# yangdongchao/Text-to-sound-Synthesis

Hardware: NVIDIA H100
Metric: clips/sec (10s audio, 100 diffusion steps) (higher is better)
Workload: dtype f16x3

## Files before the change

text-to-sound-synthesis_b200/csrc/attention_tc_split.cu:

```cuda
#include "common.cuh"
#include "diffsound_b200.h"
#include <cuda_fp16.h>

namespace dsb {
namespace {
constexpr int SP_HD = 64;
constexpr int SP_KMAX = 288;
constexpr int SP_MAX_WARPS = 12;

struct SpParams {
  int B, H, Lq, Lk, kpad, box_rows, n_box;
  int slabs, slabs_per_cta;
  const __half* q;
  long long ldq;
  int q_lo_col, k_lo_col, v_lo_col;
  long long ldo, o_lo_off;
  __half* o;
  float scale_log2e;
};

__device__ __forceinline__ float sp_ex2(float x) {
  float y;
  asm("ex2.approx.ftz.f32 %0, %1;" : "=f"(y) : "f"(x));
  return y;
}

__device__ __forceinline__ uint32_t sp_sw128(int r, int chunk) { return r * 128 + ((chunk ^ (r & 7)) << 4); }
__device__ __forceinline__ void sp_ldsm_x4(uint32_t (&r)[4], const uint8_t* p) {
  asm volatile("ldmatrix.sync.aligned.m8n8.x4.shared.b16 {%0,%1,%2,%3}, [%4];" : "=r"(r[0]), "=r"(r[1]), "=r"(r[2]), "=r"(r[3]) : "r"(smem_u32(p)));
}
__device__ __forceinline__ void sp_ldsm_x4_t(uint32_t (&r)[4], const uint8_t* p) {
  asm volatile("ldmatrix.sync.aligned.m8n8.x4.trans.shared.b16 {%0,%1,%2,%3}, [%4];" : "=r"(r[0]), "=r"(r[1]), "=r"(r[2]), "=r"(r[3]) : "r"(smem_u32(p)));
}
__device__ __forceinline__ void sp_mma(float (&d)[4], const uint32_t (&a)[4], uint32_t b0, uint32_t b1) {
  asm volatile("mma.sync.aligned.m16n8k16.row.col.f32.f16.f16.f32 {%0,%1,%2,%3}, {%4,%5,%6,%7}, {%8,%9}, {%0,%1,%2,%3};"
               : "+f"(d[0]), "+f"(d[1]), "+f"(d[2]), "+f"(d[3])
               : "r"(a[0]), "r"(a[1]), "r"(a[2]), "r"(a[3]), "r"(b0), "r"(b1));
}
__device__ __forceinline__ void sp_pack_pair(float a, float b, uint32_t& hi, uint32_t& lo) {
  const __half2 h = __floats2half2_rn(a, b);
  const __half2 l = __floats2half2_rn(a - __low2float(h), b - __high2float(h));
  hi = *reinterpret_cast<const uint32_t*>(&h);
  lo = *reinterpret_cast<const uint32_t*>(&l);
}
__device__ __forceinline__ void sp_remainder_rows(const SpParams& p, const uint8_t* sKh, const uint8_t* sKl, const uint8_t* sVh, const uint8_t* sVl, int b, int h,
                                                  int row0, int lane) {
  const int g = lane >> 2, t = lane & 3;
  const __half* qb = p.q + (long long)b * p.Lq * p.ldq + h * SP_HD;
  uint32_t ah[4][4], al[4][4];
#pragma unroll
  for (int ks = 0; ks < 4; ++ks) {
    const int ra = row0 + g, rb = row0 + g + 8, c = ks * 16 + 2 * t;
    const __half* pa = qb + (long long)ra * p.ldq + c;
    const __half* pb = qb + (long long)rb * p.ldq + c;
    ah[ks][0] = ra < p.Lq ? *reinterpret_cast<const uint32_t*>(pa) : 0u;
    ah[ks][1] = rb < p.Lq ? *reinterpret_cast<const uint32_t*>(pb) : 0u;
    ah[ks][2] = ra < p.Lq ? *reinterpret_cast<const uint32_t*>(pa + 8) : 0u;
    ah[ks][3] = rb < p.Lq ? *reinterpret_cast<const uint32_t*>(pb + 8) : 0u;
    al[ks][0] = ra < p.Lq ? *reinterpret_cast<const uint32_t*>(pa + p.q_lo_col) : 0u;
    al[ks][1] = rb < p.Lq ? *reinterpret_cast<const uint32_t*>(pb + p.q_lo_col) : 0u;
    al[ks][2] = ra < p.Lq ? *reinterpret_cast<const uint32_t*>(pa + p.q_lo_col + 8) : 0u;
    al[ks][3] = rb < p.Lq ? *reinterpret_cast<const uint32_t*>(pb + p.q_lo_col + 8) : 0u;
  }
  float m0 = -INFINITY, m1 = -INFINITY, l0 = 0.f, l1 = 0.f;
  float oacc[8][4];
#pragma unroll
  for (int i = 0; i < 8; ++i) oacc[i][0] = oacc[i][1] = oacc[i][2] = oacc[i][3] = 0.f;
  for (int kc = 0; kc * 64 < p.kpad; ++kc) {
    const int keys_left = p.Lk - kc * 64;
    if (keys_left <= 0) break;
    const int n_live = keys_left >= 64 ? 8 : (keys_left + 7) >> 3;
    float s[8][4];
#pragma unroll
    for (int nt = 0; nt < 8; ++nt) {
      s[nt][0] = s[nt][1] = s[nt][2] = s[nt][3] = 0.f;
      if (nt >= n_live) continue;
      const int row = kc * 64 + nt * 8 + (lane & 7);
      uint32_t kh[4], kl[4];
#pragma unroll
      for (int half = 0; half < 2; ++half) {
        sp_ldsm_x4(kh, sKh + sp_sw128(row, 4 * half + (lane >> 3)));
        sp_ldsm_x4(kl, sKl + sp_sw128(row, 4 * half + (lane >> 3)));
        sp_mma(s[nt], al[2 * half], kh[0], kh[1]);
        sp_mma(s[nt], al[2 * half + 1], kh[2], kh[3]);
        sp_mma(s[nt], ah[2 * half], kl[0], kl[1]);
        sp_mma(s[nt], ah[2 * half + 1], kl[2], kl[3]);
        sp_mma(s[nt], ah[2 * half], kh[0], kh[1]);
        sp_mma(s[nt], ah[2 * half + 1], kh[2], kh[3]);
      }
    }
    float mx0 = -INFINITY, mx1 = -INFINITY;
#pragma unroll
    for (int nt = 0; nt < 8; ++nt) {
      const int key = kc * 64 + nt * 8 + 2 * t;
      if (key >= p.Lk) { s[nt][0] = -INFINITY; s[nt][2] = -INFINITY; }
      if (key + 1 >= p.Lk) { s[nt][1] = -INFINITY; s[nt][3] = -INFINITY; }
      mx0 = fmaxf(mx0, fmaxf(s[nt][0], s[nt][1]));
      mx1 = fmaxf(mx1, fmaxf(s[nt][2], s[nt][3]));
    }
    mx0 = fmaxf(mx0, __shfl_xor_sync(0xffffffffu, mx0, 1)); mx0 = fmaxf(mx0, __shfl_xor_sync(0xffffffffu, mx0, 2));
    mx1 = fmaxf(mx1, __shfl_xor_sync(0xffffffffu, mx1, 1)); mx1 = fmaxf(mx1, __shfl_xor_sync(0xffffffffu, mx1, 2));
    const float mn0 = fmaxf(m0, mx0), mn1 = fmaxf(m1, mx1);
    const float c0 = sp_ex2((m0 - mn0) * p.scale_log2e), c1 = sp_ex2((m1 - mn1) * p.scale_log2e);
    const float ms0 = mn0 * p.scale_log2e, ms1 = mn1 * p.scale_log2e;
    m0 = mn0; m1 = mn1;
    l0 *= c0; l1 *= c1;
#pragma unroll
    for (int nd = 0; nd < 8; ++nd) { oacc[nd][0] *= c0; oacc[nd][1] *= c0; oacc[nd][2] *= c1; oacc[nd][3] *= c1; }
#pragma unroll
    for (int nt = 0; nt < 8; ++nt) {
      s[nt][0] = sp_ex2(fmaf(s[nt][0], p.scale_log2e, -ms0)); s[nt][1] = sp_ex2(fmaf(s[nt][1], p.scale_log2e, -ms0));
      s[nt][2] = sp_ex2(fmaf(s[nt][2], p.scale_log2e, -ms1)); s[nt][3] = sp_ex2(fmaf(s[nt][3], p.scale_log2e, -ms1));
      l0 += s[nt][0] + s[nt][1];
      l1 += s[nt][2] + s[nt][3];
    }
#pragma unroll
    for (int kk = 0; kk < 4; ++kk) {
      if (kk * 2 >= n_live) continue;
      uint32_t ph[4], pl[4];
      sp_pack_pair(s[2 * kk][0], s[2 * kk][1], ph[0], pl[0]);
      sp_pack_pair(s[2 * kk][2], s[2 * kk][3], ph[1], pl[1]);
      sp_pack_pair(s[2 * kk + 1][0], s[2 * kk + 1][1], ph[2], pl[2]);
      sp_pack_pair(s[2 * kk + 1][2], s[2 * kk + 1][3], ph[3], pl[3]);
      const int row = kc * 64 + kk * 16 + (lane & 7) + 8 * ((lane >> 3) & 1);
#pragma unroll
      for (int np = 0; np < 4; ++np) {
        uint32_t vh[4], vl[4];
        sp_ldsm_x4_t(vh, sVh + sp_sw128(row, 2 * np + (lane >> 4)));
        sp_ldsm_x4_t(vl, sVl + sp_sw128(row, 2 * np + (lane >> 4)));
        sp_mma(oacc[2 * np], pl, vh[0], vh[1]);
        sp_mma(oacc[2 * np + 1], pl, vh[2], vh[3]);
        sp_mma(oacc[2 * np], ph, vl[0], vl[1]);
        sp_mma(oacc[2 * np + 1], ph, vl[2], vl[3]);
        sp_mma(oacc[2 * np], ph, vh[0], vh[1]);
        sp_mma(oacc[2 * np + 1], ph, vh[2], vh[3]);
      }
    }
  }
  l0 += __shfl_xor_sync(0xffffffffu, l0, 1); l0 += __shfl_xor_sync(0xffffffffu, l0, 2);
  l1 += __shfl_xor_sync(0xffffffffu, l1, 1); l1 += __shfl_xor_sync(0xffffffffu, l1, 2);
  const float i0 = 1.0f / l0, i1 = 1.0f / l1;
  const int ra = row0 + g, rb = row0 + g + 8;
  __half* ob = p.o + (long long)b * p.Lq * p.ldo + h * SP_HD;
#pragma unroll
  for (int nd = 0; nd < 8; ++nd) {
    uint32_t hi, lo;
    if (ra < p.Lq) {
      sp_pack_pair(oacc[nd][0] * i0, oacc[nd][1] * i0, hi, lo);
      *reinterpret_cast<uint32_t*>(ob + (long long)ra * p.ldo + nd * 8 + 2 * t) = hi;
      *reinterpret_cast<uint32_t*>(ob + (long long)ra * p.ldo + p.o_lo_off + nd * 8 + 2 * t) = lo;
    }
    if (rb < p.Lq) {
      sp_pack_pair(oacc[nd][2] * i1, oacc[nd][3] * i1, hi, lo);
      *reinterpret_cast<uint32_t*>(ob + (long long)rb * p.ldo + nd * 8 + 2 * t) = hi;
      *reinterpret_cast<uint32_t*>(ob + (long long)rb * p.ldo + p.o_lo_off + nd * 8 + 2 * t) = lo;
    }
  }
}

__global__ void __launch_bounds__(SP_MAX_WARPS * 32, 1)
attention_tc_split_kernel(const __grid_constant__ CUtensorMap map_k, const __grid_constant__ CUtensorMap map_v, const __grid_constant__ SpParams p) {
  extern __shared__ uint8_t smem_raw[];
  uint8_t* smem = reinterpret_cast<uint8_t*>((reinterpret_cast<uintptr_t>(smem_raw) + 1023) & ~uintptr_t(1023));
  const int kv_bytes = p.kpad * 128;
  uint8_t* sKh = smem;
  uint8_t* sKl = sKh + kv_bytes;
  uint8_t* sVh = sKl + kv_bytes;
  uint8_t* sVl = sVh + kv_bytes;
  uint64_t* kv_full = reinterpret_cast<uint64_t*>(sVl + kv_bytes);
  const int u = blockIdx.x, b = u / p.H, h = u - b * p.H;
  const int warp = threadIdx.x >> 5, lane = threadIdx.x & 31;

  if (threadIdx.x == 0) {
    mbar_init(kv_full, 1);
    fence_barrier_init();
    prefetch_tmap(&map_k); prefetch_tmap(&map_v);
  }
  __syncthreads();
  pdl_wait();
  pdl_trigger();
  if (threadIdx.x == 0) {
    mbar_arrive_expect_tx(kv_full, 4 * kv_bytes);
    for (int bx = 0; bx < p.n_box; ++bx) {
      const int r = b * p.Lk + bx * p.box_rows, off = bx * p.box_rows * 128;
      tma_load_3d(&map_k, kv_full, sKh + off, h * SP_HD, r, 0);
      tma_load_3d(&map_k, kv_full, sKl + off, p.k_lo_col + h * SP_HD, r, 0);
      tma_load_3d(&map_v, kv_full, sVh + off, h * SP_HD, r, 0);
      tma_load_3d(&map_v, kv_full, sVl + off, p.v_lo_col + h * SP_HD, r, 0);
    }
  }
  mbar_wait(kv_full, 0);
  const int s0 = blockIdx.y * p.slabs_per_cta, s1 = min(p.slabs, s0 + p.slabs_per_cta);
  for (int sl = s0 + warp; sl < s1; sl += blockDim.x >> 5) sp_remainder_rows(p, sKh, sKl, sVh, sVl, b, h, sl * 16, lane);
}
}
}

extern "C" int dsb_attention_tc_split(const void* q, long long ldq, long long q_lo_off, const void* k, long long ldk, long long k_lo_off, const void* v,
                                      long long ldv, long long v_lo_off, void* o, long long ldo, long long o_lo_off, int B, int H, int Lq, int Lk,
                                      float scale, void* stream) {
  using namespace dsb;
  DSB_REQUIRE(B > 0 && H > 0 && Lq > 0 && Lk > 0 && Lk <= SP_KMAX, "dsb_attention_tc_split: need 0 < Lk <= %d", SP_KMAX);
  DSB_REQUIRE(ldo % 8 == 0 && o_lo_off % 8 == 0 && (reinterpret_cast<uintptr_t>(o) & 15) == 0, "dsb_attention_tc_split: o must be 16-byte aligned, ldo / o_lo_off %% 8 == 0");
  DSB_REQUIRE(q_lo_off >= (long long)H * SP_HD && k_lo_off >= (long long)H * SP_HD && v_lo_off >= (long long)H * SP_HD && o_lo_off >= (long long)H * SP_HD,
              "dsb_attention_tc_split: the lo halves must not overlap the hi halves");
  DSB_REQUIRE(q_lo_off + (long long)H * SP_HD <= ldq && k_lo_off + (long long)H * SP_HD <= ldk && v_lo_off + (long long)H * SP_HD <= ldv,
              "dsb_attention_tc_split: lo halves must lie inside a row (lo_off + H*64 <= ld)");
  DSB_REQUIRE(ldq % 2 == 0 && q_lo_off % 2 == 0 && (reinterpret_cast<uintptr_t>(q) & 3) == 0, "dsb_attention_tc_split: q must be 4-byte aligned");
  SpParams p{};
  p.B = B; p.H = H; p.Lq = Lq; p.Lk = Lk;
  p.kpad = (Lk + 31) & ~31;
  p.q = (const __half*)q; p.ldq = ldq;
  p.n_box = p.kpad > 256 ? 2 : 1;
  p.box_rows = p.kpad / p.n_box;
  DSB_REQUIRE(p.box_rows % 8 == 0, "dsb_attention_tc_split: internal box size");
  p.q_lo_col = (int)q_lo_off; p.k_lo_col = (int)k_lo_off; p.v_lo_col = (int)v_lo_off;
  p.ldo = ldo; p.o_lo_off = o_lo_off; p.o = (__half*)o;
  p.scale_log2e = scale * 1.4426950408889634f;
  p.slabs = (Lq + 15) / 16;
  const int ny = (p.slabs + SP_MAX_WARPS - 1) / SP_MAX_WARPS;
  p.slabs_per_cta = (p.slabs + ny - 1) / ny;
  CUtensorMap mk, mv;
  if (make_operand_map(&mk, k, DSB_DTYPE_F16, k_lo_off + (long long)H * SP_HD, (long long)B * Lk, 1, ldk, 0, p.box_rows)) return 3;
  if (make_operand_map(&mv, v, DSB_DTYPE_F16, v_lo_off + (long long)H * SP_HD, (long long)B * Lk, 1, ldv, 0, p.box_rows)) return 3;
  const int smem = 4 * p.kpad * 128 + 8 + 1024;
  static int attr_smem = 0;
  if (smem > attr_smem) {
    DSB_CHECK_CUDA(cudaFuncSetAttribute(attention_tc_split_kernel, cudaFuncAttributeMaxDynamicSharedMemorySize, smem));
    attr_smem = smem;
  }
  DSB_CHECK_CUDA(launch_pdl(attention_tc_split_kernel, dim3(B * H, ny), dim3(p.slabs_per_cta * 32), smem, (cudaStream_t)stream, mk, mv, p));
  return 0;
}
```

text-to-sound-synthesis_b200/csrc/wgmma.cuh:

```cuda
#pragma once
#include "common.cuh"
#include "diffsound_b200.h"

namespace dsb {

template <int KIND, int TA, int TB>
__device__ __forceinline__ void wgmma_m64n128(float (&d)[64], uint64_t da, uint64_t db, uint32_t scale_d) {
  static_assert(KIND != DSB_DTYPE_TF32 || (TA == 0 && TB == 0), "tf32 wgmma takes K-major operands only");
  if constexpr (KIND == DSB_DTYPE_TF32) {
    asm volatile(
        "{\n\t.reg .pred p;\n\tsetp.ne.b32 p, %66, 0;\n\t"
        "wgmma.mma_async.sync.aligned.m64n128k8.f32.tf32.tf32 "
        "{%0, %1, %2, %3, %4, %5, %6, %7, %8, %9, %10, %11, %12, %13, %14, %15, %16, %17, %18, %19, %20, %21, %22, %23, %24, %25, %26, %27, %28, %29, %30, %31, %32, %33, %34, %35, %36, %37, %38, %39, %40, %41, %42, %43, %44, %45, %46, %47, %48, %49, %50, %51, %52, %53, %54, %55, %56, %57, %58, %59, %60, %61, %62, %63}, "
        "%64, %65, p, 1, 1;\n\t}"
        : "+f"(d[0]), "+f"(d[1]), "+f"(d[2]), "+f"(d[3]), "+f"(d[4]), "+f"(d[5]), "+f"(d[6]), "+f"(d[7]), "+f"(d[8]), "+f"(d[9]), "+f"(d[10]), "+f"(d[11]), "+f"(d[12]), "+f"(d[13]), "+f"(d[14]), "+f"(d[15]), "+f"(d[16]), "+f"(d[17]), "+f"(d[18]), "+f"(d[19]), "+f"(d[20]), "+f"(d[21]), "+f"(d[22]), "+f"(d[23]), "+f"(d[24]), "+f"(d[25]), "+f"(d[26]), "+f"(d[27]), "+f"(d[28]), "+f"(d[29]), "+f"(d[30]), "+f"(d[31]), "+f"(d[32]), "+f"(d[33]), "+f"(d[34]), "+f"(d[35]), "+f"(d[36]), "+f"(d[37]), "+f"(d[38]), "+f"(d[39]), "+f"(d[40]), "+f"(d[41]), "+f"(d[42]), "+f"(d[43]), "+f"(d[44]), "+f"(d[45]), "+f"(d[46]), "+f"(d[47]), "+f"(d[48]), "+f"(d[49]), "+f"(d[50]), "+f"(d[51]), "+f"(d[52]), "+f"(d[53]), "+f"(d[54]), "+f"(d[55]), "+f"(d[56]), "+f"(d[57]), "+f"(d[58]), "+f"(d[59]), "+f"(d[60]), "+f"(d[61]), "+f"(d[62]), "+f"(d[63])
        : "l"(da), "l"(db), "r"(scale_d));
  } else if constexpr (KIND == DSB_DTYPE_BF16) {
    asm volatile(
        "{\n\t.reg .pred p;\n\tsetp.ne.b32 p, %66, 0;\n\t"
        "wgmma.mma_async.sync.aligned.m64n128k16.f32.bf16.bf16 "
        "{%0, %1, %2, %3, %4, %5, %6, %7, %8, %9, %10, %11, %12, %13, %14, %15, %16, %17, %18, %19, %20, %21, %22, %23, %24, %25, %26, %27, %28, %29, %30, %31, %32, %33, %34, %35, %36, %37, %38, %39, %40, %41, %42, %43, %44, %45, %46, %47, %48, %49, %50, %51, %52, %53, %54, %55, %56, %57, %58, %59, %60, %61, %62, %63}, "
        "%64, %65, p, 1, 1, %67, %68;\n\t}"
        : "+f"(d[0]), "+f"(d[1]), "+f"(d[2]), "+f"(d[3]), "+f"(d[4]), "+f"(d[5]), "+f"(d[6]), "+f"(d[7]), "+f"(d[8]), "+f"(d[9]), "+f"(d[10]), "+f"(d[11]), "+f"(d[12]), "+f"(d[13]), "+f"(d[14]), "+f"(d[15]), "+f"(d[16]), "+f"(d[17]), "+f"(d[18]), "+f"(d[19]), "+f"(d[20]), "+f"(d[21]), "+f"(d[22]), "+f"(d[23]), "+f"(d[24]), "+f"(d[25]), "+f"(d[26]), "+f"(d[27]), "+f"(d[28]), "+f"(d[29]), "+f"(d[30]), "+f"(d[31]), "+f"(d[32]), "+f"(d[33]), "+f"(d[34]), "+f"(d[35]), "+f"(d[36]), "+f"(d[37]), "+f"(d[38]), "+f"(d[39]), "+f"(d[40]), "+f"(d[41]), "+f"(d[42]), "+f"(d[43]), "+f"(d[44]), "+f"(d[45]), "+f"(d[46]), "+f"(d[47]), "+f"(d[48]), "+f"(d[49]), "+f"(d[50]), "+f"(d[51]), "+f"(d[52]), "+f"(d[53]), "+f"(d[54]), "+f"(d[55]), "+f"(d[56]), "+f"(d[57]), "+f"(d[58]), "+f"(d[59]), "+f"(d[60]), "+f"(d[61]), "+f"(d[62]), "+f"(d[63])
        : "l"(da), "l"(db), "r"(scale_d), "n"(TA), "n"(TB));
  } else {
    asm volatile(
        "{\n\t.reg .pred p;\n\tsetp.ne.b32 p, %66, 0;\n\t"
        "wgmma.mma_async.sync.aligned.m64n128k16.f32.f16.f16 "
        "{%0, %1, %2, %3, %4, %5, %6, %7, %8, %9, %10, %11, %12, %13, %14, %15, %16, %17, %18, %19, %20, %21, %22, %23, %24, %25, %26, %27, %28, %29, %30, %31, %32, %33, %34, %35, %36, %37, %38, %39, %40, %41, %42, %43, %44, %45, %46, %47, %48, %49, %50, %51, %52, %53, %54, %55, %56, %57, %58, %59, %60, %61, %62, %63}, "
        "%64, %65, p, 1, 1, %67, %68;\n\t}"
        : "+f"(d[0]), "+f"(d[1]), "+f"(d[2]), "+f"(d[3]), "+f"(d[4]), "+f"(d[5]), "+f"(d[6]), "+f"(d[7]), "+f"(d[8]), "+f"(d[9]), "+f"(d[10]), "+f"(d[11]), "+f"(d[12]), "+f"(d[13]), "+f"(d[14]), "+f"(d[15]), "+f"(d[16]), "+f"(d[17]), "+f"(d[18]), "+f"(d[19]), "+f"(d[20]), "+f"(d[21]), "+f"(d[22]), "+f"(d[23]), "+f"(d[24]), "+f"(d[25]), "+f"(d[26]), "+f"(d[27]), "+f"(d[28]), "+f"(d[29]), "+f"(d[30]), "+f"(d[31]), "+f"(d[32]), "+f"(d[33]), "+f"(d[34]), "+f"(d[35]), "+f"(d[36]), "+f"(d[37]), "+f"(d[38]), "+f"(d[39]), "+f"(d[40]), "+f"(d[41]), "+f"(d[42]), "+f"(d[43]), "+f"(d[44]), "+f"(d[45]), "+f"(d[46]), "+f"(d[47]), "+f"(d[48]), "+f"(d[49]), "+f"(d[50]), "+f"(d[51]), "+f"(d[52]), "+f"(d[53]), "+f"(d[54]), "+f"(d[55]), "+f"(d[56]), "+f"(d[57]), "+f"(d[58]), "+f"(d[59]), "+f"(d[60]), "+f"(d[61]), "+f"(d[62]), "+f"(d[63])
        : "l"(da), "l"(db), "r"(scale_d), "n"(TA), "n"(TB));
  }
}

}
```

Before: 8.421.

## Rewrite split-precision attention as warp-specialized WGMMA kernel with TMA K/V ring

Replaces the mma.sync/ldmatrix attention, which loaded all of K/V for a (batch, head) into shared memory at once, with a persistent warp-specialized kernel. A producer warp streams Q tiles and 64-key K/V chunks through a 4-stage TMA ring. Two consumer warpgroups run 3-term split-f16 QK^T and PV with wgmma m64n64 and stage the output through shared memory for coalesced stores. This drops the Lk<=288 limit and is meant to raise tensor-core throughput. In exchange, each chunk waits on wgmma before softmax, so MMA and softmax do not overlap within a warpgroup, and Q/O now need 16-byte alignment for TMA.

```diff
diff --git a/text-to-sound-synthesis_b200/csrc/attention_tc_split.cu b/text-to-sound-synthesis_b200/csrc/attention_tc_split.cu
--- a/text-to-sound-synthesis_b200/csrc/attention_tc_split.cu
+++ b/text-to-sound-synthesis_b200/csrc/attention_tc_split.cu
@@ -1,197 +1,233 @@
 #include "common.cuh"
 #include "diffsound_b200.h"
+#include "wgmma.cuh"
 #include <cuda_fp16.h>
 
 namespace dsb {
 namespace {
-constexpr int SP_HD = 64;
-constexpr int SP_KMAX = 288;
-constexpr int SP_MAX_WARPS = 12;
-
-struct SpParams {
-  int B, H, Lq, Lk, kpad, box_rows, n_box;
-  int slabs, slabs_per_cta;
-  const __half* q;
-  long long ldq;
+constexpr int AT_HD = 64;
+constexpr int AT_TILE = 64 * 128;
+constexpr int AT_STAGES = 4;
+constexpr int AT_STAGE_BYTES = 4 * AT_TILE;
+constexpr int AT_Q_BYTES = 2 * AT_TILE;
+constexpr int AT_THREADS = 384;
+constexpr int AT_SMEM = AT_STAGES * AT_STAGE_BYTES + 4 * AT_Q_BYTES + 4 * AT_STAGES * 8 + 1024;
+
+struct AtParams {
+  int H, Lq, Lk;
+  int n_chunks, n_tiles, n_pairs, n_units;
   int q_lo_col, k_lo_col, v_lo_col;
   long long ldo, o_lo_off;
   __half* o;
   float scale_log2e;
 };
 
-__device__ __forceinline__ float sp_ex2(float x) {
+__device__ __forceinline__ float at_ex2(float x) {
   float y;
   asm("ex2.approx.ftz.f32 %0, %1;" : "=f"(y) : "f"(x));
   return y;
 }
-
-__device__ __forceinline__ uint32_t sp_sw128(int r, int chunk) { return r * 128 + ((chunk ^ (r & 7)) << 4); }
-__device__ __forceinline__ void sp_ldsm_x4(uint32_t (&r)[4], const uint8_t* p) {
-  asm volatile("ldmatrix.sync.aligned.m8n8.x4.shared.b16 {%0,%1,%2,%3}, [%4];" : "=r"(r[0]), "=r"(r[1]), "=r"(r[2]), "=r"(r[3]) : "r"(smem_u32(p)));
-}
-__device__ __forceinline__ void sp_ldsm_x4_t(uint32_t (&r)[4], const uint8_t* p) {
-  asm volatile("ldmatrix.sync.aligned.m8n8.x4.trans.shared.b16 {%0,%1,%2,%3}, [%4];" : "=r"(r[0]), "=r"(r[1]), "=r"(r[2]), "=r"(r[3]) : "r"(smem_u32(p)));
-}
-__device__ __forceinline__ void sp_mma(float (&d)[4], const uint32_t (&a)[4], uint32_t b0, uint32_t b1) {
-  asm volatile("mma.sync.aligned.m16n8k16.row.col.f32.f16.f16.f32 {%0,%1,%2,%3}, {%4,%5,%6,%7}, {%8,%9}, {%0,%1,%2,%3};"
-               : "+f"(d[0]), "+f"(d[1]), "+f"(d[2]), "+f"(d[3])
-               : "r"(a[0]), "r"(a[1]), "r"(a[2]), "r"(a[3]), "r"(b0), "r"(b1));
-}
-__device__ __forceinline__ void sp_pack_pair(float a, float b, uint32_t& hi, uint32_t& lo) {
+__device__ __forceinline__ void at_pack_pair(float a, float b, uint32_t& hi, uint32_t& lo) {
   const __half2 h = __floats2half2_rn(a, b);
   const __half2 l = __floats2half2_rn(a - __low2float(h), b - __high2float(h));
   hi = *reinterpret_cast<const uint32_t*>(&h);
   lo = *reinterpret_cast<const uint32_t*>(&l);
 }
-__device__ __forceinline__ void sp_remainder_rows(const SpParams& p, const uint8_t* sKh, const uint8_t* sKl, const uint8_t* sVh, const uint8_t* sVl, int b, int h,
-                                                  int row0, int lane) {
-  const int g = lane >> 2, t = lane & 3;
-  const __half* qb = p.q + (long long)b * p.Lq * p.ldq + h * SP_HD;
-  uint32_t ah[4][4], al[4][4];
-#pragma unroll
-  for (int ks = 0; ks < 4; ++ks) {
-    const int ra = row0 + g, rb = row0 + g + 8, c = ks * 16 + 2 * t;
-    const __half* pa = qb + (long long)ra * p.ldq + c;
-    const __half* pb = qb + (long long)rb * p.ldq + c;
-    ah[ks][0] = ra < p.Lq ? *reinterpret_cast<const uint32_t*>(pa) : 0u;
-    ah[ks][1] = rb < p.Lq ? *reinterpret_cast<const uint32_t*>(pb) : 0u;
-    ah[ks][2] = ra < p.Lq ? *reinterpret_cast<const uint32_t*>(pa + 8) : 0u;
-    ah[ks][3] = rb < p.Lq ? *reinterpret_cast<const uint32_t*>(pb + 8) : 0u;
-    al[ks][0] = ra < p.Lq ? *reinterpret_cast<const uint32_t*>(pa + p.q_lo_col) : 0u;
-    al[ks][1] = rb < p.Lq ? *reinterpret_cast<const uint32_t*>(pb + p.q_lo_col) : 0u;
-    al[ks][2] = ra < p.Lq ? *reinterpret_cast<const uint32_t*>(pa + p.q_lo_col + 8) : 0u;
-    al[ks][3] = rb < p.Lq ? *reinterpret_cast<const uint32_t*>(pb + p.q_lo_col + 8) : 0u;
-  }
+
+__device__ __forceinline__ void at_tile(const AtParams& p, uint8_t* ring, uint64_t* full, uint64_t* empty, int& stage, uint32_t& phase, uint8_t* sq,
+                                        int b, int h, int tile, int wg, int wq, int lane) {
+  const int t = lane & 3;
+  const uint32_t sq_u = smem_u32(sq);
+  float o[32], s[32], part[32];
+#pragma unroll
+  for (int i = 0; i < 32; ++i) o[i] = 0.f;
   float m0 = -INFINITY, m1 = -INFINITY, l0 = 0.f, l1 = 0.f;
-  float oacc[8][4];
-#pragma unroll
-  for (int i = 0; i < 8; ++i) oacc[i][0] = oacc[i][1] = oacc[i][2] = oacc[i][3] = 0.f;
-  for (int kc = 0; kc * 64 < p.kpad; ++kc) {
-    const int keys_left = p.Lk - kc * 64;
-    if (keys_left <= 0) break;
-    const int n_live = keys_left >= 64 ? 8 : (keys_left + 7) >> 3;
-    float s[8][4];
-#pragma unroll
-    for (int nt = 0; nt < 8; ++nt) {
-      s[nt][0] = s[nt][1] = s[nt][2] = s[nt][3] = 0.f;
-      if (nt >= n_live) continue;
-      const int row = kc * 64 + nt * 8 + (lane & 7);
-      uint32_t kh[4], kl[4];
-#pragma unroll
-      for (int half = 0; half < 2; ++half) {
-        sp_ldsm_x4(kh, sKh + sp_sw128(row, 4 * half + (lane >> 3)));
-        sp_ldsm_x4(kl, sKl + sp_sw128(row, 4 * half + (lane >> 3)));
-        sp_mma(s[nt], al[2 * half], kh[0], kh[1]);
-        sp_mma(s[nt], al[2 * half + 1], kh[2], kh[3]);
-        sp_mma(s[nt], ah[2 * half], kl[0], kl[1]);
-        sp_mma(s[nt], ah[2 * half + 1], kl[2], kl[3]);
-        sp_mma(s[nt], ah[2 * half], kh[0], kh[1]);
-        sp_mma(s[nt], ah[2 * half + 1], kh[2], kh[3]);
+  for (int c = 0; c < p.n_chunks; ++c) {
+    mbar_wait(&full[stage], phase);
+    const uint32_t sk = smem_u32(ring + stage * AT_STAGE_BYTES);
+    wgmma_fence_regs(s);
+    wgmma_fence();
+#pragma unroll
+    for (int k = 0; k < 4; ++k) {
+      const uint64_t dqh = make_sw128_kmajor_desc(sq_u) + 2 * k, dql = make_sw128_kmajor_desc(sq_u + AT_TILE) + 2 * k;
+      const uint64_t dkh = make_sw128_kmajor_desc(sk) + 2 * k, dkl = make_sw128_kmajor_desc(sk + AT_TILE) + 2 * k;
+      wgmma_m64n64_f16_ss<0, 0>(s, dql, dkh, k != 0 ? 1u : 0u);
+      wgmma_m64n64_f16_ss<0, 0>(s, dqh, dkl, 1u);
+      wgmma_m64n64_f16_ss<0, 0>(s, dqh, dkh, 1u);
+    }
+    wgmma_commit();
+    wgmma_wait<0>();
+    wgmma_fence_regs(s);
+
+    if ((c + 1) * 64 > p.Lk) {
+#pragma unroll
+      for (int j = 0; j < 8; ++j) {
+        const int key = c * 64 + j * 8 + 2 * t;
+        if (key >= p.Lk) { s[4 * j] = -INFINITY; s[4 * j + 2] = -INFINITY; }
+        if (key + 1 >= p.Lk) { s[4 * j + 1] = -INFINITY; s[4 * j + 3] = -INFINITY; }
       }
     }
     float mx0 = -INFINITY, mx1 = -INFINITY;
 #pragma unroll
-    for (int nt = 0; nt < 8; ++nt) {
-      const int key = kc * 64 + nt * 8 + 2 * t;
-      if (key >= p.Lk) { s[nt][0] = -INFINITY; s[nt][2] = -INFINITY; }
-      if (key + 1 >= p.Lk) { s[nt][1] = -INFINITY; s[nt][3] = -INFINITY; }
-      mx0 = fmaxf(mx0, fmaxf(s[nt][0], s[nt][1]));
-      mx1 = fmaxf(mx1, fmaxf(s[nt][2], s[nt][3]));
+    for (int j = 0; j < 8; ++j) {
+      mx0 = fmaxf(mx0, fmaxf(s[4 * j], s[4 * j + 1]));
+      mx1 = fmaxf(mx1, fmaxf(s[4 * j + 2], s[4 * j + 3]));
     }
     mx0 = fmaxf(mx0, __shfl_xor_sync(0xffffffffu, mx0, 1)); mx0 = fmaxf(mx0, __shfl_xor_sync(0xffffffffu, mx0, 2));
     mx1 = fmaxf(mx1, __shfl_xor_sync(0xffffffffu, mx1, 1)); mx1 = fmaxf(mx1, __shfl_xor_sync(0xffffffffu, mx1, 2));
     const float mn0 = fmaxf(m0, mx0), mn1 = fmaxf(m1, mx1);
-    const float c0 = sp_ex2((m0 - mn0) * p.scale_log2e), c1 = sp_ex2((m1 - mn1) * p.scale_log2e);
+    const float c0 = at_ex2((m0 - mn0) * p.scale_log2e), c1 = at_ex2((m1 - mn1) * p.scale_log2e);
     const float ms0 = mn0 * p.scale_log2e, ms1 = mn1 * p.scale_log2e;
     m0 = mn0; m1 = mn1;
     l0 *= c0; l1 *= c1;
 #pragma unroll
-    for (int nd = 0; nd < 8; ++nd) { oacc[nd][0] *= c0; oacc[nd][1] *= c0; oacc[nd][2] *= c1; oacc[nd][3] *= c1; }
-#pragma unroll
-    for (int nt = 0; nt < 8; ++nt) {
-      s[nt][0] = sp_ex2(fmaf(s[nt][0], p.scale_log2e, -ms0)); s[nt][1] = sp_ex2(fmaf(s[nt][1], p.scale_log2e, -ms0));
-      s[nt][2] = sp_ex2(fmaf(s[nt][2], p.scale_log2e, -ms1)); s[nt][3] = sp_ex2(fmaf(s[nt][3], p.scale_log2e, -ms1));
-      l0 += s[nt][0] + s[nt][1];
-      l1 += s[nt][2] + s[nt][3];
-    }
+    for (int j = 0; j < 8; ++j) { o[4 * j] *= c0; o[4 * j + 1] *= c0; o[4 * j + 2] *= c1; o[4 * j + 3] *= c1; }
+#pragma unroll
+    for (int j = 0; j < 8; ++j) {
+      s[4 * j] = at_ex2(fmaf(s[4 * j], p.scale_log2e, -ms0)); s[4 * j + 1] = at_ex2(fmaf(s[4 * j + 1], p.scale_log2e, -ms0));
+      s[4 * j + 2] = at_ex2(fmaf(s[4 * j + 2], p.scale_log2e, -ms1)); s[4 * j + 3] = at_ex2(fmaf(s[4 * j + 3], p.scale_log2e, -ms1));
+      l0 += s[4 * j] + s[4 * j + 1];
+      l1 += s[4 * j + 2] + s[4 * j + 3];
+    }
+    uint32_t ph[4][4], pl[4][4];
 #pragma unroll
     for (int kk = 0; kk < 4; ++kk) {
-      if (kk * 2 >= n_live) continue;
-      uint32_t ph[4], pl[4];
-      sp_pack_pair(s[2 * kk][0], s[2 * kk][1], ph[0], pl[0]);
-      sp_pack_pair(s[2 * kk][2], s[2 * kk][3], ph[1], pl[1]);
-      sp_pack_pair(s[2 * kk + 1][0], s[2 * kk + 1][1], ph[2], pl[2]);
-      sp_pack_pair(s[2 * kk + 1][2], s[2 * kk + 1][3], ph[3], pl[3]);
-      const int row = kc * 64 + kk * 16 + (lane & 7) + 8 * ((lane >> 3) & 1);
-#pragma unroll
-      for (int np = 0; np < 4; ++np) {
-        uint32_t vh[4], vl[4];
-        sp_ldsm_x4_t(vh, sVh + sp_sw128(row, 2 * np + (lane >> 4)));
-        sp_ldsm_x4_t(vl, sVl + sp_sw128(row, 2 * np + (lane >> 4)));
-        sp_mma(oacc[2 * np], pl, vh[0], vh[1]);
-        sp_mma(oacc[2 * np + 1], pl, vh[2], vh[3]);
-        sp_mma(oacc[2 * np], ph, vl[0], vl[1]);
-        sp_mma(oacc[2 * np + 1], ph, vl[2], vl[3]);
-        sp_mma(oacc[2 * np], ph, vh[0], vh[1]);
-        sp_mma(oacc[2 * np + 1], ph, vh[2], vh[3]);
-      }
-    }
-  }
+      at_pack_pair(s[8 * kk], s[8 * kk + 1], ph[kk][0], pl[kk][0]);
+      at_pack_pair(s[8 * kk + 2], s[8 * kk + 3], ph[kk][1], pl[kk][1]);
+      at_pack_pair(s[8 * kk + 4], s[8 * kk + 5], ph[kk][2], pl[kk][2]);
+      at_pack_pair(s[8 * kk + 6], s[8 * kk + 7], ph[kk][3], pl[kk][3]);
+    }
+    wgmma_fence_regs(part);
+    wgmma_fence();
+#pragma unroll
+    for (int kk = 0; kk < 4; ++kk) {
+      const uint64_t dvh = make_sw128_desc(sk + 2 * AT_TILE, AT_TILE) + 128 * kk, dvl = make_sw128_desc(sk + 3 * AT_TILE, AT_TILE) + 128 * kk;
+      wgmma_m64n64_f16_rs<1>(part, pl[kk], dvh, kk != 0 ? 1u : 0u);
+      wgmma_m64n64_f16_rs<1>(part, ph[kk], dvl, 1u);
+      wgmma_m64n64_f16_rs<1>(part, ph[kk], dvh, 1u);
+    }
+    wgmma_commit();
+    wgmma_wait<0>();
+    wgmma_fence_regs(part);
+    if (lane == 0) mbar_arrive(&empty[stage]);
+#pragma unroll
+    for (int i = 0; i < 32; ++i) o[i] += part[i];
+    if (++stage == AT_STAGES) { stage = 0; phase ^= 1; }
+  }
+
   l0 += __shfl_xor_sync(0xffffffffu, l0, 1); l0 += __shfl_xor_sync(0xffffffffu, l0, 2);
   l1 += __shfl_xor_sync(0xffffffffu, l1, 1); l1 += __shfl_xor_sync(0xffffffffu, l1, 2);
-  const float i0 = 1.0f / l0, i1 = 1.0f / l1;
-  const int ra = row0 + g, rb = row0 + g + 8;
-  __half* ob = p.o + (long long)b * p.Lq * p.ldo + h * SP_HD;
-#pragma unroll
-  for (int nd = 0; nd < 8; ++nd) {
+  const float i0 = __fdividef(1.0f, l0), i1 = __fdividef(1.0f, l1);
+  named_bar_sync(1 + wg, 128);
+  const int r0 = wq * 16 + (lane >> 2), r1 = r0 + 8;
+#pragma unroll
+  for (int j = 0; j < 8; ++j) {
     uint32_t hi, lo;
-    if (ra < p.Lq) {
-      sp_pack_pair(oacc[nd][0] * i0, oacc[nd][1] * i0, hi, lo);
-      *reinterpret_cast<uint32_t*>(ob + (long long)ra * p.ldo + nd * 8 + 2 * t) = hi;
-      *reinterpret_cast<uint32_t*>(ob + (long long)ra * p.ldo + p.o_lo_off + nd * 8 + 2 * t) = lo;
-    }
-    if (rb < p.Lq) {
-      sp_pack_pair(oacc[nd][2] * i1, oacc[nd][3] * i1, hi, lo);
-      *reinterpret_cast<uint32_t*>(ob + (long long)rb * p.ldo + nd * 8 + 2 * t) = hi;
-      *reinterpret_cast<uint32_t*>(ob + (long long)rb * p.ldo + p.o_lo_off + nd * 8 + 2 * t) = lo;
-    }
-  }
-}
-
-__global__ void __launch_bounds__(SP_MAX_WARPS * 32, 1)
-attention_tc_split_kernel(const __grid_constant__ CUtensorMap map_k, const __grid_constant__ CUtensorMap map_v, const __grid_constant__ SpParams p) {
+    at_pack_pair(o[4 * j] * i0, o[4 * j + 1] * i0, hi, lo);
+    *reinterpret_cast<uint32_t*>(sq + r0 * 128 + ((j ^ (r0 & 7)) << 4) + 4 * t) = hi;
+    *reinterpret_cast<uint32_t*>(sq + AT_TILE + r0 * 128 + ((j ^ (r0 & 7)) << 4) + 4 * t) = lo;
+    at_pack_pair(o[4 * j + 2] * i1, o[4 * j + 3] * i1, hi, lo);
+    *reinterpret_cast<uint32_t*>(sq + r1 * 128 + ((j ^ (r1 & 7)) << 4) + 4 * t) = hi;
+    *reinterpret_cast<uint32_t*>(sq + AT_TILE + r1 * 128 + ((j ^ (r1 & 7)) << 4) + 4 * t) = lo;
+  }
+  named_bar_sync(1 + wg, 128);
+  const int ct = wq * 32 + lane;
+  __half* ob = p.o + (long long)b * p.Lq * p.ldo + h * AT_HD;
+#pragma unroll
+  for (int i = 0; i < 8; ++i) {
+    const int idx = ct + 128 * i, half = idx >> 9, r = (idx >> 3) & 63, ch = idx & 7;
+    const int row = tile * 64 + r;
+    if (row < p.Lq)
+      *reinterpret_cast<uint4*>(ob + (long long)row * p.ldo + half * p.o_lo_off + ch * 8) =
+          *reinterpret_cast<const uint4*>(sq + half * AT_TILE + r * 128 + ((ch ^ (r & 7)) << 4));
+  }
+  fence_proxy_async_smem();
+}
+
+__global__ void __launch_bounds__(AT_THREADS, 1)
+attention_tc_split_kernel(const __grid_constant__ CUtensorMap map_q, const __grid_constant__ CUtensorMap map_k, const __grid_constant__ CUtensorMap map_v,
+                          const __grid_constant__ AtParams p) {
   extern __shared__ uint8_t smem_raw[];
   uint8_t* smem = reinterpret_cast<uint8_t*>((reinterpret_cast<uintptr_t>(smem_raw) + 1023) & ~uintptr_t(1023));
-  const int kv_bytes = p.kpad * 128;
-  uint8_t* sKh = smem;
-  uint8_t* sKl = sKh + kv_bytes;
-  uint8_t* sVh = sKl + kv_bytes;
-  uint8_t* sVl = sVh + kv_bytes;
-  uint64_t* kv_full = reinterpret_cast<uint64_t*>(sVl + kv_bytes);
-  const int u = blockIdx.x, b = u / p.H, h = u - b * p.H;
+  uint8_t* ring = smem;
+  uint8_t* qbuf = ring + AT_STAGES * AT_STAGE_BYTES;
+  uint64_t* full = reinterpret_cast<uint64_t*>(qbuf + 4 * AT_Q_BYTES);
+  uint64_t* empty = full + AT_STAGES;
+  uint64_t* q_full = empty + AT_STAGES;
+  uint64_t* q_empty = q_full + 4;
   const int warp = threadIdx.x >> 5, lane = threadIdx.x & 31;
 
   if (threadIdx.x == 0) {
-    mbar_init(kv_full, 1);
+    for (int s = 0; s < AT_STAGES; ++s) {
+      mbar_init(&full[s], 1);
+      mbar_init(&empty[s], 8);
+    }
+    for (int i = 0; i < 4; ++i) {
+      mbar_init(&q_full[i], 1);
+      mbar_init(&q_empty[i], 4);
+    }
     fence_barrier_init();
-    prefetch_tmap(&map_k); prefetch_tmap(&map_v);
+    prefetch_tmap(&map_q); prefetch_tmap(&map_k); prefetch_tmap(&map_v);
   }
   __syncthreads();
   pdl_wait();
   pdl_trigger();
-  if (threadIdx.x == 0) {
-    mbar_arrive_expect_tx(kv_full, 4 * kv_bytes);
-    for (int bx = 0; bx < p.n_box; ++bx) {
-      const int r = b * p.Lk + bx * p.box_rows, off = bx * p.box_rows * 128;
-      tma_load_3d(&map_k, kv_full, sKh + off, h * SP_HD, r, 0);
-      tma_load_3d(&map_k, kv_full, sKl + off, p.k_lo_col + h * SP_HD, r, 0);
-      tma_load_3d(&map_v, kv_full, sVh + off, h * SP_HD, r, 0);
-      tma_load_3d(&map_v, kv_full, sVl + off, p.v_lo_col + h * SP_HD, r, 0);
-    }
-  }
-  mbar_wait(kv_full, 0);
-  const int s0 = blockIdx.y * p.slabs_per_cta, s1 = min(p.slabs, s0 + p.slabs_per_cta);
-  for (int sl = s0 + warp; sl < s1; sl += blockDim.x >> 5) sp_remainder_rows(p, sKh, sKl, sVh, sVl, b, h, sl * 16, lane);
+
+  if (warp < 4) {
+    setmaxnreg_dec<40>();
+    if (threadIdx.x == 0) {
+      int stage = 0, qn[2] = {0, 0};
+      uint32_t phase = 0;
+      for (int u = blockIdx.x; u < p.n_units; u += gridDim.x) {
+        const int bh = u / p.n_pairs, pair = u - bh * p.n_pairs, b = bh / p.H, h = bh - b * p.H;
+#pragma unroll
+        for (int w = 0; w < 2; ++w) {
+          const int tile = 2 * pair + w;
+          if (tile >= p.n_tiles) continue;
+          const int q = 2 * w + (qn[w] & 1);
+          mbar_wait(&q_empty[q], ((qn[w] >> 1) & 1) ^ 1);
+          mbar_arrive_expect_tx(&q_full[q], AT_Q_BYTES);
+          uint8_t* dst = qbuf + q * AT_Q_BYTES;
+          tma_load_3d(&map_q, &q_full[q], dst, h * AT_HD, tile * 64, b);
+          tma_load_3d(&map_q, &q_full[q], dst + AT_TILE, p.q_lo_col + h * AT_HD, tile * 64, b);
+          ++qn[w];
+        }
+        for (int c = 0; c < p.n_chunks; ++c) {
+          mbar_wait(&empty[stage], phase ^ 1);
+          mbar_arrive_expect_tx(&full[stage], AT_STAGE_BYTES);
+          uint8_t* st = ring + stage * AT_STAGE_BYTES;
+          tma_load_3d(&map_k, &full[stage], st, h * AT_HD, c * 64, b);
+          tma_load_3d(&map_k, &full[stage], st + AT_TILE, p.k_lo_col + h * AT_HD, c * 64, b);
+          tma_load_3d(&map_v, &full[stage], st + 2 * AT_TILE, h * AT_HD, c * 64, b);
+          tma_load_3d(&map_v, &full[stage], st + 3 * AT_TILE, p.v_lo_col + h * AT_HD, c * 64, b);
+          if (++stage == AT_STAGES) { stage = 0; phase ^= 1; }
+        }
+      }
+    }
+  } else {
+    setmaxnreg_inc<232>();
+    const int wg = (warp >> 2) - 1, wq = warp & 3;
+    int stage = 0, qn = 0;
+    uint32_t phase = 0;
+    for (int u = blockIdx.x; u < p.n_units; u += gridDim.x) {
+      const int bh = u / p.n_pairs, pair = u - bh * p.n_pairs, b = bh / p.H, h = bh - b * p.H;
+      const int tile = 2 * pair + wg;
+      if (tile < p.n_tiles) {
+        const int q = 2 * wg + (qn & 1);
+        mbar_wait(&q_full[q], (qn >> 1) & 1);
+        at_tile(p, ring, full, empty, stage, phase, qbuf + q * AT_Q_BYTES, b, h, tile, wg, wq, lane);
+        __syncwarp();
+        if (lane == 0) mbar_arrive(&q_empty[q]);
+        ++qn;
+      } else {
+        for (int c = 0; c < p.n_chunks; ++c) {
+          mbar_wait(&full[stage], phase);
+          if (lane == 0) mbar_arrive(&empty[stage]);
+          if (++stage == AT_STAGES) { stage = 0; phase ^= 1; }
+        }
+      }
+    }
+  }
 }
 }
 }
@@ -200,35 +236,34 @@
                                       long long ldv, long long v_lo_off, void* o, long long ldo, long long o_lo_off, int B, int H, int Lq, int Lk,
                                       float scale, void* stream) {
   using namespace dsb;
-  DSB_REQUIRE(B > 0 && H > 0 && Lq > 0 && Lk > 0 && Lk <= SP_KMAX, "dsb_attention_tc_split: need 0 < Lk <= %d", SP_KMAX);
+  DSB_REQUIRE(B > 0 && H > 0 && Lq > 0 && Lk > 0, "dsb_attention_tc_split: need B, H, Lq, Lk > 0");
   DSB_REQUIRE(ldo % 8 == 0 && o_lo_off % 8 == 0 && (reinterpret_cast<uintptr_t>(o) & 15) == 0, "dsb_attention_tc_split: o must be 16-byte aligned, ldo / o_lo_off %% 8 == 0");
-  DSB_REQUIRE(q_lo_off >= (long long)H * SP_HD && k_lo_off >= (long long)H * SP_HD && v_lo_off >= (long long)H * SP_HD && o_lo_off >= (long long)H * SP_HD,
+  DSB_REQUIRE(q_lo_off >= (long long)H * AT_HD && k_lo_off >= (long long)H * AT_HD && v_lo_off >= (long long)H * AT_HD && o_lo_off >= (long long)H * AT_HD,
               "dsb_attention_tc_split: the lo halves must not overlap the hi halves");
-  DSB_REQUIRE(q_lo_off + (long long)H * SP_HD <= ldq && k_lo_off + (long long)H * SP_HD <= ldk && v_lo_off + (long long)H * SP_HD <= ldv,
+  DSB_REQUIRE(q_lo_off + (long long)H * AT_HD <= ldq && k_lo_off + (long long)H * AT_HD <= ldk && v_lo_off + (long long)H * AT_HD <= ldv,
               "dsb_attention_tc_split: lo halves must lie inside a row (lo_off + H*64 <= ld)");
-  DSB_REQUIRE(ldq % 2 == 0 && q_lo_off % 2 == 0 && (reinterpret_cast<uintptr_t>(q) & 3) == 0, "dsb_attention_tc_split: q must be 4-byte aligned");
-  SpParams p{};
-  p.B = B; p.H = H; p.Lq = Lq; p.Lk = Lk;
-  p.kpad = (Lk + 31) & ~31;
-  p.q = (const __half*)q; p.ldq = ldq;
-  p.n_box = p.kpad > 256 ? 2 : 1;
-  p.box_rows = p.kpad / p.n_box;
-  DSB_REQUIRE(p.box_rows % 8 == 0, "dsb_attention_tc_split: internal box size");
+  DSB_REQUIRE(ldq % 8 == 0 && (reinterpret_cast<uintptr_t>(q) & 15) == 0, "dsb_attention_tc_split: q must be 16-byte aligned, ldq %% 8 == 0 (TMA)");
+  AtParams p{};
+  p.H = H; p.Lq = Lq; p.Lk = Lk;
+  p.n_chunks = (Lk + 63) / 64;
+  p.n_tiles = (Lq + 63) / 64;
+  p.n_pairs = (p.n_tiles + 1) / 2;
+  const long long units = (long long)B * H * p.n_pairs;
+  DSB_REQUIRE(units < (1LL << 31), "dsb_attention_tc_split: too many (batch, head, tile pair) units");
+  p.n_units = (int)units;
   p.q_lo_col = (int)q_lo_off; p.k_lo_col = (int)k_lo_off; p.v_lo_col = (int)v_lo_off;
   p.ldo = ldo; p.o_lo_off = o_lo_off; p.o = (__half*)o;
   p.scale_log2e = scale * 1.4426950408889634f;
-  p.slabs = (Lq + 15) / 16;
-  const int ny = (p.slabs + SP_MAX_WARPS - 1) / SP_MAX_WARPS;
-  p.slabs_per_cta = (p.slabs + ny - 1) / ny;
-  CUtensorMap mk, mv;
-  if (make_operand_map(&mk, k, DSB_DTYPE_F16, k_lo_off + (long long)H * SP_HD, (long long)B * Lk, 1, ldk, 0, p.box_rows)) return 3;
-  if (make_operand_map(&mv, v, DSB_DTYPE_F16, v_lo_off + (long long)H * SP_HD, (long long)B * Lk, 1, ldv, 0, p.box_rows)) return 3;
-  const int smem = 4 * p.kpad * 128 + 8 + 1024;
-  static int attr_smem = 0;
-  if (smem > attr_smem) {
-    DSB_CHECK_CUDA(cudaFuncSetAttribute(attention_tc_split_kernel, cudaFuncAttributeMaxDynamicSharedMemorySize, smem));
-    attr_smem = smem;
-  }
-  DSB_CHECK_CUDA(launch_pdl(attention_tc_split_kernel, dim3(B * H, ny), dim3(p.slabs_per_cta * 32), smem, (cudaStream_t)stream, mk, mv, p));
+  CUtensorMap mq, mk, mv;
+  if (make_operand_map(&mq, q, DSB_DTYPE_F16, q_lo_off + (long long)H * AT_HD, Lq, B, ldq, (long long)Lq * ldq, 64)) return 3;
+  if (make_operand_map(&mk, k, DSB_DTYPE_F16, k_lo_off + (long long)H * AT_HD, Lk, B, ldk, (long long)Lk * ldk, 64)) return 3;
+  if (make_operand_map(&mv, v, DSB_DTYPE_F16, v_lo_off + (long long)H * AT_HD, Lk, B, ldv, (long long)Lk * ldv, 64)) return 3;
+  static bool attr_set = false;
+  if (!attr_set) {
+    DSB_CHECK_CUDA(cudaFuncSetAttribute(attention_tc_split_kernel, cudaFuncAttributeMaxDynamicSharedMemorySize, AT_SMEM));
+    attr_set = true;
+  }
+  const int grid = min(p.n_units, sm_count());
+  DSB_CHECK_CUDA(launch_pdl(attention_tc_split_kernel, dim3(grid), dim3(AT_THREADS), AT_SMEM, (cudaStream_t)stream, mq, mk, mv, p));
   return 0;
 }
diff --git a/text-to-sound-synthesis_b200/csrc/wgmma.cuh b/text-to-sound-synthesis_b200/csrc/wgmma.cuh
--- a/text-to-sound-synthesis_b200/csrc/wgmma.cuh
+++ b/text-to-sound-synthesis_b200/csrc/wgmma.cuh
@@ -34,4 +34,26 @@
   }
 }
 
+template <int TA, int TB>
+__device__ __forceinline__ void wgmma_m64n64_f16_ss(float (&d)[32], uint64_t da, uint64_t db, uint32_t scale_d) {
+  asm volatile(
+      "{\n\t.reg .pred p;\n\tsetp.ne.b32 p, %34, 0;\n\t"
+      "wgmma.mma_async.sync.aligned.m64n64k16.f32.f16.f16 "
+      "{%0, %1, %2, %3, %4, %5, %6, %7, %8, %9, %10, %11, %12, %13, %14, %15, %16, %17, %18, %19, %20, %21, %22, %23, %24, %25, %26, %27, %28, %29, %30, %31}, "
+      "%32, %33, p, 1, 1, %35, %36;\n\t}"
+      : "+f"(d[0]), "+f"(d[1]), "+f"(d[2]), "+f"(d[3]), "+f"(d[4]), "+f"(d[5]), "+f"(d[6]), "+f"(d[7]), "+f"(d[8]), "+f"(d[9]), "+f"(d[10]), "+f"(d[11]), "+f"(d[12]), "+f"(d[13]), "+f"(d[14]), "+f"(d[15]), "+f"(d[16]), "+f"(d[17]), "+f"(d[18]), "+f"(d[19]), "+f"(d[20]), "+f"(d[21]), "+f"(d[22]), "+f"(d[23]), "+f"(d[24]), "+f"(d[25]), "+f"(d[26]), "+f"(d[27]), "+f"(d[28]), "+f"(d[29]), "+f"(d[30]), "+f"(d[31])
+      : "l"(da), "l"(db), "r"(scale_d), "n"(TA), "n"(TB));
 }
+
+template <int TB>
+__device__ __forceinline__ void wgmma_m64n64_f16_rs(float (&d)[32], const uint32_t (&a)[4], uint64_t db, uint32_t scale_d) {
+  asm volatile(
+      "{\n\t.reg .pred p;\n\tsetp.ne.b32 p, %37, 0;\n\t"
+      "wgmma.mma_async.sync.aligned.m64n64k16.f32.f16.f16 "
+      "{%0, %1, %2, %3, %4, %5, %6, %7, %8, %9, %10, %11, %12, %13, %14, %15, %16, %17, %18, %19, %20, %21, %22, %23, %24, %25, %26, %27, %28, %29, %30, %31}, "
+      "{%32, %33, %34, %35}, %36, p, 1, 1, %38;\n\t}"
+      : "+f"(d[0]), "+f"(d[1]), "+f"(d[2]), "+f"(d[3]), "+f"(d[4]), "+f"(d[5]), "+f"(d[6]), "+f"(d[7]), "+f"(d[8]), "+f"(d[9]), "+f"(d[10]), "+f"(d[11]), "+f"(d[12]), "+f"(d[13]), "+f"(d[14]), "+f"(d[15]), "+f"(d[16]), "+f"(d[17]), "+f"(d[18]), "+f"(d[19]), "+f"(d[20]), "+f"(d[21]), "+f"(d[22]), "+f"(d[23]), "+f"(d[24]), "+f"(d[25]), "+f"(d[26]), "+f"(d[27]), "+f"(d[28]), "+f"(d[29]), "+f"(d[30]), "+f"(d[31])
+      : "r"(a[0]), "r"(a[1]), "r"(a[2]), "r"(a[3]), "l"(db), "r"(scale_d), "n"(TB));
+}
+
+}
```

Result: faster. 8.800, median of 6 (+4.5%).
